# jdidion/atropos

Hardware: AMD Instinct MI355X
Metric: reads/s (whole node) 150 bp SE adapter-align (higher is better)
Workload: dtype int32

## Files before the change

### atropos_amd/csrc/piece_filter.hpp

```cpp
#ifndef ATR_PIECE_FILTER_HPP
#define ATR_PIECE_FILTER_HPP

#include "fast_work.hpp"
#include "pack_fast.hpp"

namespace atr {

#ifndef ATR_PIECE_PREFETCH_EARLY
#define ATR_PIECE_PREFETCH_EARLY 1
#endif
#ifndef ATR_PIECE_STASH
#define ATR_PIECE_STASH 1
#endif
#ifndef ATR_PIECE_WAVES
#if defined(ATR_SPEC) && defined(ATR_SPEC_ASCII)
#define ATR_PIECE_WAVES(NW) 2
#elif defined(ATR_SPEC)
#define ATR_PIECE_WAVES(NW) ((NW) <= 6 ? 4 : 3)
#else
#define ATR_PIECE_WAVES(NW) ((NW) <= 6 ? 4 : (NW) <= 8 ? 3 : 2)
#endif
#endif

constexpr int PIECE_QF = 2;
template <bool B> struct PieceBool { static constexpr bool value = B; };

__device__ __forceinline__ int lane_rank(uint64_t mask) {
    return (int)__builtin_amdgcn_mbcnt_hi((uint32_t)(mask >> 32), __builtin_amdgcn_mbcnt_lo((uint32_t)mask, 0u));
}

__device__ __forceinline__ void piece_emit(bool active, long long r, uint32_t ww, const uint32_t (&rec)[4], int m, uint4 *out,
                                           uint2 *list, uint4 *ldata, const uint32_t *nibs, int j0, uint32_t *s_lcur, uint32_t *s_hist,
                                           int nd = 8) {
    const bool open = active && window_valid(ww);
    if (active && !open) out[r] = make_uint4(rec[0], rec[1], rec[2], rec[3]);
    const uint64_t om = __ballot(open);
    if (om != 0ull) {
        uint32_t base = 0u;
        if ((threadIdx.x & 63) == 0) base = atomicAdd(s_lcur, (uint32_t)__popcll(om));
        base = __builtin_amdgcn_readfirstlane(base);
        const int lane = threadIdx.x & 63;
        const int off = window_lo(ww) - j0;
        const bool dense = nibs != nullptr && off >= 0 && off < 64 && band_stream_dwords(m) <= 8;
        if (open) {
            const uint32_t slot = base + (uint32_t)lane_rank(om);
            list[slot] = make_uint2((uint32_t)r, dense ? ww : (ww | PIECE_NODENSE));
            atomicAdd(&s_hist[window_bin(ww, m, true)], 1u);
            if (dense) {
                const int z = off >> 3;
                const uint32_t sh = 4u * (uint32_t)(off & 7);
                uint32_t raw[9], d[8];
#pragma unroll
                for (int k = 0; k < 9; ++k) raw[k] = z + k < nd ? nibs[(z + k) * 64 + lane] : 0u;
#pragma unroll
                for (int k = 0; k < 8; ++k) d[k] = sh ? ((raw[k] >> sh) | (raw[k + 1] << (32u - sh))) : raw[k];
                ldata[2 * (size_t)slot] = make_uint4(d[0], d[1], d[2], d[3]);
                ldata[2 * (size_t)slot + 1] = make_uint4(d[4], d[5], d[6], d[7]);
            }
        }
    }
}

template <int NW, bool RAGGED, int WW = 2>
__device__ __forceinline__ void piece_filter_body(const LocateParams &p, const FilterParams &fp_arg, const PieceParams &pp_arg,
                                                  const uint4 *__restrict__ planes, const int32_t *__restrict__ lens,
                                                  long long nreads, int max_len, uint4 *__restrict__ out, FastWork wk,
                                                  const uint8_t *__restrict__ ascii = nullptr, const uint8_t *tab = nullptr) {
#ifdef ATR_SPEC
    if (!RAGGED) max_len = spec::N;
#endif
#ifdef ATR_SPEC_ASCII
    static_assert(NW <= 8, "the fused ASCII entry keeps pass B's window in the LDS stash");
    constexpr int STRIDE = ATR_SPEC_STRIDE;
    constexpr int NPC = (15 + 64 * STRIDE + 1023) / 1024;
    constexpr int STAGE_BYTES = (64 * STRIDE + PACK_STAGE_SLACK + 15) & ~15;
    __shared__ __attribute__((aligned(16))) uint8_t s_stage[4][STAGE_BYTES];
    __shared__ uint8_t s_tab[256];
    s_tab[threadIdx.x] = tab[threadIdx.x];
    uint4 *planes_out = const_cast<uint4 *>(planes);
    const uint8_t *buf_end = ascii + nreads * STRIDE;
#endif
    const int n = RAGGED ? 32 * NW : max_len;
    __shared__ uint2 s_peq[16];
    __shared__ uint32_t s_spread[4][256];
    __shared__ uint32_t s_hist[FILTER_BINS];
    __shared__ uint32_t s_lcur, s_wcnt;
    constexpr int PW = 32 * WW, ND = 4 * WW;
#ifdef ATR_SPEC
    constexpr bool WIDE_OK = true;
#else
    constexpr bool WIDE_OK = WW == 3;
#endif
    static_assert(WW == 2 || WW == 3, "windows of 64 or 96 columns");
    __shared__ uint32_t s_nibs[4][ND][64];
    __shared__ uint32_t s_queue[4][PIECE_QF][64];
    constexpr bool STASH = ATR_PIECE_STASH != 0 && NW <= 8;
    __shared__ uint4 s_stash[STASH ? 4 : 1][STASH ? NW : 1][64];
    const Uniform u = make_uniform(p, round_up_rows_dev(p.m));
#ifndef ATR_SPEC
    __shared__ PieceParams s_pp;
    __shared__ FilterParams s_fp;
    for (int i = threadIdx.x; i < (int)(sizeof(PieceParams) / 4); i += 256) ((uint32_t *)&s_pp)[i] = ((const uint32_t *)&pp_arg)[i];
    for (int i = threadIdx.x; i < (int)(sizeof(FilterParams) / 4); i += 256) ((uint32_t *)&s_fp)[i] = ((const uint32_t *)&fp_arg)[i];
    const PieceParams &pp = s_pp;
    const FilterParams &fp = s_fp;
#else
    const PieceParams &pp = pp_arg;
    const FilterParams &fp = fp_arg;
#endif
    if (threadIdx.x < 16) s_peq[threadIdx.x] = make_uint2((uint32_t)fp_arg.peq[threadIdx.x], (uint32_t)(fp_arg.peq[threadIdx.x] >> 32));
    if (threadIdx.x < FILTER_BINS) s_hist[threadIdx.x] = 0;
    if (threadIdx.x == 0) { s_lcur = 0; s_wcnt = 0; }
    piece_spread_fill(s_spread);
    __syncthreads();

    const int lane = threadIdx.x & 63, wave = __builtin_amdgcn_readfirstlane((int)(threadIdx.x >> 6));
    const int mf = fp_arg.rows, T = u.m - mf;
    const uint32_t kreg = (uint32_t)u.k;
    const long long ntiles = (nreads + 63) >> 6;
    long long t0, t1;
    block_tiles(ntiles, t0, t1, wk.nused);
    uint2 *list = wk.tmp + t0 * 64;
    uint4 *ldata = wk.tdata + t0 * 128;
    uint32_t *wlist = wk.wide + t0 * 64;
    uint32_t (*queue)[64] = s_queue[wave];
    uint32_t *nibs = &s_nibs[wave][0][0];
    uint4 (*stash)[64] = s_stash[STASH ? wave : 0];

    auto pass_b = [&](int count) __attribute__((always_inline)) {
        const bool act = lane < count;
        const long long r = (long long)queue[0][lane];
        const uint32_t meta = queue[1][lane];
        const int j_e = act ? (int)(meta & 1023u) : 0, need = act ? (int)((meta >> 10) & 127u) : 0;
        const int nr = RAGGED ? (act ? (int)(meta >> 17) : 0) : max_len;
        uint32_t wp[4][WW];
        {
            const int b0 = j_e - PW + (STASH && RAGGED ? 32 * NW - nr : 0), w0 = b0 >> 5;
            uint4 g[WW + 1];
#pragma unroll
            for (int i = 0; i <= WW; ++i) g[i] = make_uint4(0u, 0u, 0u, 0u);
            if constexpr (STASH) {
                if (act) {
#pragma unroll
                    for (int i = 0; i <= WW; ++i) if (w0 + i >= 0 && w0 + i < NW) g[i] = stash[w0 + i][lane];
                }
            } else {
#ifndef ATR_X_NOGATHER
                const uint4 *tcur = planes + ((size_t)(r >> 6) * NW) * 64 + (r & 63);
                if (act) {
#pragma unroll
                    for (int i = 0; i <= WW; ++i) if (w0 + i >= 0 && w0 + i < NW) g[i] = tcur[(size_t)(w0 + i) * 64];
                }
#endif
            }
            const uint32_t sh = (uint32_t)(b0 & 31);
#pragma unroll
            for (int i = 0; i < WW; ++i) {
                wp[0][i] = __builtin_amdgcn_alignbit(g[i + 1].x, g[i].x, sh);
                wp[1][i] = __builtin_amdgcn_alignbit(g[i + 1].y, g[i].y, sh);
                wp[2][i] = __builtin_amdgcn_alignbit(g[i + 1].z, g[i].z, sh);
                wp[3][i] = __builtin_amdgcn_alignbit(g[i + 1].w, g[i].w, sh);
            }
        }
        const int W = min(PW, (wave_max_i32(need) + 7) & ~7);
        const int dw0 = ND - (W >> 3);
        uint32_t nb[ND];
#pragma unroll
        for (int d = 0; d < ND; ++d) {
            nb[d] = 0u;
            if (d >= dw0 - 1) nb[d] = piece_nibbles(s_spread, wp[0][d >> 2], wp[1][d >> 2], wp[2][d >> 2], wp[3][d >> 2], d & 3);
            nibs[d * 64 + lane] = nb[d];
        }
        const auto sweep_decide = [&](auto wc) __attribute__((always_inline)) {
        constexpr bool WD = decltype(wc)::value;
        FilterState F;
        filter_init(F, u, mf, WD);
        int vstart = 0;
        if (u.sr) {
            const bool zero0 = j_e - W <= 0;
            Uniform uf = u;
            uf.sr = false;
            FilterState G;
            filter_init(G, uf, mf, WD);
            if (!zero0) { F.pvl = G.pvl; F.pvh = G.pvh; F.score = G.score; }
            vstart = zero0 ? PW - j_e : 0;
        }
        uint2 ea[8], eb[8];
#pragma unroll
        for (int d = 0; d < ND; ++d) {
            if (d < dw0) continue;
            uint2 (&e)[8] = (d & 1) ? eb : ea;
            if (d == dw0) fetch_peq8(s_peq, nb[d], e);
            if (d + 1 < ND) fetch_peq8(s_peq, nb[d + 1], (d & 1) ? ea : eb);
            if (u.sr) {
#pragma unroll
                for (int b = 0; b < 8; ++b) if (8 * d + b < vstart) { e[b].x = ~0u; e[b].y = ~0u; }
            }
#pragma unroll
            for (int b = 0; b < 8; ++b) filter_step<WD>(F, e[b].x, e[b].y, kreg);
            if ((d & 3) == 3 && d + 1 < ND) filter_fold(F, j_e - PW + 8 * (d + 1), mf, kreg);
        }
        filter_fold(F, j_e, mf, kreg);
        uint32_t rec[4];
        const auto tm = [&](int jp) {
            const int rp = max(0, jp - (j_e - PW));
            return filter_tail_cmp(fp, T, rp, [&](int z) { return z < ND ? nibs[z * 64 + lane] : 0u; });
        };
        const auto dg = [&](int d) -> uint64_t {
            if constexpr (WW != 2 || WD) return ~0ull;
            const int o = d - (j_e - PW);
            if (o < 0 || o + u.m > PW) return ~0ull;
            uint64_t eq = 0ull;
#pragma unroll
            for (int c = 0; c < 4; ++c) {
                uint32_t lo = wp[c][0], hi = wp[c][1];
#pragma unroll
                for (int q = 0; q < 4; ++q) if (q != c && !fp.and_mode) { lo &= ~wp[q][0]; hi &= ~wp[q][1]; }
                eq |= ((((uint64_t)hi << 32) | lo) >> o) & fp.rowsel[c];
            }
            return ~eq & (u.m >= 64 ? ~0ull : (1ull << u.m) - 1ull);
        };
        const uint32_t ww = filter_decide_tm<WD>(F, u, fp, tm, nr, rec, 0, j_e == nr, dg, j_e - need, j_e < nr ? j_e - u.m : -0x10000);
        piece_emit(act, r, ww, rec, u.m, out, list, ldata, nibs, j_e - PW, &s_lcur, s_hist, ND);
        };
        if (mf > 32) {
            if constexpr (WIDE_OK) sweep_decide(PieceBool<true>{});
        } else {
            sweep_decide(PieceBool<false>{});
        }
    };

    int qn = 0;

#ifdef ATR_SPEC_ASCII
    uint4 ax[NPC];
    const auto ascii_edge = [&](long long tile) {
        const uint8_t *src = ascii + tile * 64 * STRIDE;
        const uint8_t *al = src - ((uintptr_t)src & 15);
        const long long need = (long long)((uintptr_t)src & 15) + (nreads - tile * 64 < 64 ? nreads - tile * 64 : 64) * STRIDE;
        return al < ascii || al + ((need + 15) & ~15ll) > buf_end;
    };
    const auto ascii_request = [&](long long tile) {
        if (ascii_edge(tile)) return;
        const uint8_t *src = ascii + tile * 64 * STRIDE;
        const uint8_t *al = src - ((uintptr_t)src & 15);
        const long long need = (long long)((uintptr_t)src & 15) + (nreads - tile * 64 < 64 ? nreads - tile * 64 : 64) * STRIDE;
#pragma unroll
        for (int u = 0; u < NPC; ++u) {
            const long long o = (long long)u * 1024 + (long long)lane * 16;
            ax[u] = o < need ? *(const uint4 *)(al + o) : make_uint4(0u, 0u, 0u, 0u);
        }
    };
    if (t0 + wave < t1) ascii_request(t0 + wave);
#else
    uint4 nx[NW];
    if (t0 + wave < t1) {
        const uint4 *tp = planes + (size_t)(t0 + wave) * NW * 64;
#pragma unroll
        for (int w = 0; w < NW; ++w) nx[w] = tp[w * 64 + lane];
    }
#endif
    for (long long tile = t0 + wave; tile < t1; tile += 4) {
        const long long r = tile * 64 + lane;
        const bool live = r < nreads;
        uint32_t pl[NW][4];
#ifdef ATR_SPEC_ASCII
        {
            uint8_t *stage = s_stage[wave];
            uint32_t mis;
            if (ascii_edge(tile)) {
                mis = pack_stage_tile(stage, ascii, STRIDE, nreads, tile, lane);
            } else {
                const uint8_t *src = ascii + tile * 64 * STRIDE;
                mis = (uint32_t)((uintptr_t)src & 15);
                const long long need = (long long)mis + (nreads - tile * 64 < 64 ? nreads - tile * 64 : 64) * STRIDE;
#pragma unroll
                for (int u = 0; u < NPC; ++u) {
                    const long long o = (long long)u * 1024 + (long long)lane * 16;
                    if (o < need) *(uint4 *)(stage + o) = ax[u];
                }
                __builtin_amdgcn_wave_barrier();
                __builtin_amdgcn_s_waitcnt(0);
            }
            if (tile + 4 < t1) ascii_request(tile + 4);
            __builtin_amdgcn_sched_barrier(0);
            const int np = live ? (RAGGED ? min(max(lens[r], 0), max_len) : max_len) : 0;
            const uint32_t rowoff = mis + (uint32_t)lane * (uint32_t)STRIDE;
            uint4 pk[NW];
            bool zero_seen = false;
            pack_planes_row_regs<NW>((const uint32_t *)stage, rowoff >> 2, rowoff & 3u, np, s_tab, pk, zero_seen);
            uint4 *tp = planes_out + (size_t)tile * NW * 64;
#pragma unroll
            for (int w = 0; w < NW; ++w) {
                tp[w * 64 + lane] = pk[w];
                pl[w][0] = pk[w].x; pl[w][1] = pk[w].y; pl[w][2] = pk[w].z; pl[w][3] = pk[w].w;
            }
        }
#else
#pragma unroll
        for (int w = 0; w < NW; ++w) { pl[w][0] = nx[w].x; pl[w][1] = nx[w].y; pl[w][2] = nx[w].z; pl[w][3] = nx[w].w; }
#if ATR_PIECE_PREFETCH_EARLY
        if (tile + 4 < t1) {
            const uint4 *tp = planes + (size_t)(tile + 4) * NW * 64;
#pragma unroll
            for (int w = 0; w < NW; ++w) nx[w] = tp[w * 64 + lane];
        }
        __builtin_amdgcn_sched_barrier(0);
#endif
#endif
        int nr = max_len, back = 0;
        constexpr int HWN = NW < PIECE_HEAD_WORDS ? NW : PIECE_HEAD_WORDS;
        uint32_t hpl[HWN][4];
#pragma unroll
        for (int w = 0; w < HWN; ++w)
#pragma unroll
            for (int c = 0; c < 4; ++c) hpl[w][c] = pl[w][c];
        if (RAGGED) {
            nr = live ? min(max(lens[r], 0), max_len) : 0;
            back = 32 * NW - nr;
            const int q = (back - 1) >> 5;
            const uint32_t sh = (uint32_t)(-back) & 31u;
            uint32_t x0[NW][4], x1[NW][4];
#pragma unroll
            for (int w = 0; w < NW; ++w)
#pragma unroll
                for (int c = 0; c < 4; ++c) x0[w][c] = x1[w][c] = 0u;
#pragma unroll
            for (int v = -1; v <= NW - 1; ++v) {
                const uint32_t sel = q == v ? ~0u : 0u;
#pragma unroll
                for (int w = 0; w < NW; ++w)
#pragma unroll
                    for (int c = 0; c < 4; ++c) {
                        if (w - v - 1 >= 0 && w - v - 1 < NW) x0[w][c] |= pl[w - v - 1 >= 0 && w - v - 1 < NW ? w - v - 1 : 0][c] & sel;
                        if (w - v >= 0 && w - v < NW) x1[w][c] |= pl[w - v >= 0 && w - v < NW ? w - v : 0][c] & sel;
                    }
            }
#pragma unroll
            for (int w = 0; w < NW; ++w)
#pragma unroll
                for (int c = 0; c < 4; ++c) pl[w][c] = __builtin_amdgcn_alignbit(x1[w][c], x0[w][c], sh);
        }
        uint32_t twp[4];
        {
            const int sh = n & 31;
#pragma unroll
            for (int q = 0; q < 4; ++q)
                twp[q] = sh == 0 ? pl[NW - 1][q] : __builtin_amdgcn_alignbit(pl[NW - 1][q], NW >= 2 ? pl[NW >= 2 ? NW - 2 : 0][q] : 0u, (uint32_t)sh);
        }
#ifdef ATR_SPEC
        const PieceScan S = piece_scan_spec<NW>(pl, twp, mf, T, u.k, hpl);
#else
        const PieceScan S = piece_scan<NW, (WW == 3 ? PIECE_NB : 5)>(pp, pl, twp, n, mf, T, u.k, hpl);
#endif
        const PieceTask pt = piece_task(S, back, nr, u.sr, u.m, u.k, piece_uniform(pp.head_cols));
        const bool exact = live && S.j_exact != 0 && u.m >= u.min_overlap;
        if (exact) {
            const int j = S.j_exact - back;
            out[r] = make_uint4((uint32_t)u.m << 16, (uint32_t)(j - u.m) | ((uint32_t)j << 16), (uint32_t)u.m, 0u);
        }
        const bool ovl = ATR_PIECE_OVERLAP_A != 0 && live && S.ovl != 0 && !exact;
        if (ovl) out[r] = make_uint4((uint32_t)S.ovl << 16, (uint32_t)(nr - S.ovl) | ((uint32_t)nr << 16), (uint32_t)S.ovl, 0u);
        const bool flagged = live && pt.flagged && !exact;
        if (piece_uniform(pp.aonly) != 0) {
            if (live && !flagged && !exact && !ovl) out[r] = make_uint4(0xFFFF0000u, 0u, 0u, 0u);
            const int wlo = pt.full ? 0 : pt.j_e - pt.need, whi = pt.full ? nr : pt.j_e;
            const uint32_t ww = flagged ? window_word(wlo, whi, whi == nr, u.m, false) : 0u;
            const uint32_t none[4] = {0xFFFF0000u, 0u, 0u, 0u};
            piece_emit(flagged, r, ww, none, u.m, out, list, ldata, nullptr, 0, &s_lcur, s_hist);
            continue;
        }
        const int need = pt.need;
        const bool narrow = flagged && !pt.full && need <= piece_uniform(pp.narrow), wide = flagged && !narrow;
        if (live && !flagged && !exact && !ovl) out[r] = make_uint4(0xFFFF0000u, 0u, 0u, 0u);
        const uint32_t meta = (uint32_t)pt.j_e | ((uint32_t)need << 10) | (RAGGED ? (uint32_t)nr << 17 : 0u);
        {
            const uint64_t wm = __ballot(wide);
            if (wm != 0ull) {
                uint32_t base = 0u;
                if (lane == 0) base = atomicAdd(&s_wcnt, (uint32_t)__popcll(wm));
                base = __builtin_amdgcn_readfirstlane(base);
                if (wide) wlist[(long long)base + lane_rank(wm)] = (uint32_t)r;
            }
        }
#if !ATR_PIECE_PREFETCH_EARLY && !defined(ATR_SPEC_ASCII)
        __builtin_amdgcn_sched_barrier(0);
        if (tile + 4 < t1) {
            const uint4 *tp = planes + (size_t)(tile + 4) * NW * 64;
#pragma unroll
            for (int w = 0; w < NW; ++w) nx[w] = tp[w * 64 + lane];
        }
#endif
        {
            const uint64_t nm = __ballot(narrow);
            const int cnt = (int)__popcll(nm), rank = lane_rank(nm);
            const int room = 64 - qn;
            const auto put = [&](int slot) {
                queue[0][slot] = (uint32_t)r; queue[1][slot] = meta;
                if constexpr (STASH) {
#pragma unroll
                    for (int w = 0; w < NW; ++w) stash[w][slot] = make_uint4(pl[w][0], pl[w][1], pl[w][2], pl[w][3]);
                }
            };
            if (narrow && rank < room) put(qn + rank);
            if (cnt >= room) {
                __builtin_amdgcn_fence(__ATOMIC_RELEASE, "wavefront");
                pass_b(64);
                __builtin_amdgcn_fence(__ATOMIC_RELEASE, "wavefront");
                if (narrow && rank >= room) put(rank - room);
                qn = cnt - room;
            } else {
                qn += cnt;
            }
        }
    }
    __builtin_amdgcn_fence(__ATOMIC_RELEASE, "wavefront");
    if (qn > 0) pass_b(qn);
    __threadfence_block();
    __syncthreads();
    {
        const long long total = (long long)s_wcnt;
        for (long long base = (long long)wave * 64; base < total; base += 256) {
            const bool act = base + lane < total;
            const long long r = act ? (long long)wlist[base + lane] : t0 * 64;
            const uint4 *bp = planes + ((size_t)(r >> 6) * NW) * 64 + (r & 63);
            const uint4 *tp = bp;
            const size_t tstride = 64;
            const int nl = RAGGED ? (act ? min(max(lens[r], 0), max_len) : 0) : max_len;
            const int nhi = RAGGED ? wave_max_i32(nl) : max_len;
            const auto full_sweep = [&](auto wc) __attribute__((always_inline)) {
            constexpr bool WD = decltype(wc)::value;
            FilterState F;
            filter_init(F, u, mf, WD);
            int j = 0;
#pragma clang loop unroll(disable)
            for (int c = 0; c < NW; ++c) {
                if (j >= nhi) break;
                const uint4 v = tp[(size_t)c * tstride];
#pragma clang loop unroll(disable)
                for (int d = 0; d < 4; ++d) {
                    if (j >= nhi) break;
                    uint2 e[8];
                    fetch_peq8(s_peq, piece_nibbles(s_spread, v.x, v.y, v.z, v.w, d), e);
#pragma unroll
                    for (int b = 0; b < 8; ++b)
                        if (j + b < nl) filter_step<WD>(F, e[b].x, e[b].y, kreg);
                    j += 8;
                }
                filter_fold(F, min(j, nl), mf, kreg);
            }
            uint32_t rec[4];
            const auto tm = [&](int jp) {
                return filter_tail_cmp(fp, T, jp, [&](int z) { return read_dword_planes((const uint32_t *)bp, NW, z, s_spread); });
            };
            const uint32_t ww = filter_decide_tm<WD>(F, u, fp, tm, nl, rec, 0, true);
            piece_emit(act, r, ww, rec, u.m, out, list, ldata, nullptr, 0, &s_lcur, s_hist);
            };
            if (mf > 32) {
                if constexpr (WIDE_OK) full_sweep(PieceBool<true>{});
            } else {
                full_sweep(PieceBool<false>{});
            }
        }
    }
    __syncthreads();
    fused_hist_flush(wk, s_hist);
    if (threadIdx.x == 0) wk.lcount[blockIdx.x] = s_lcur;
}

}
#endif
```

### atropos_amd/csrc/piece_kernels.hip

```cpp
#include "locate_fast.hpp"
#include "piece_filter.hpp"
#include "jit.hpp"

namespace atr {

void launch_fast_scan(FastWork wk, hipStream_t st);
int launch_fast_dp(const atr_aligner *a, const uint4 *packed, const int32_t *lens, long long nreads, int nchunks,
                   int max_len, uint4 *out, FastWork wk, const LinkedArgs *la, int idx, int count, hipStream_t st, bool planes, bool one_stream);

template <int NW, bool RAGGED, int WW>
__global__ __launch_bounds__(256) __attribute__((amdgpu_waves_per_eu(ATR_PIECE_WAVES(NW), 8))) void piece_filter_kernel(
    const LocateParams p, const FilterParams fp, const PieceParams pp, const uint4 *__restrict__ planes,
    const int32_t *__restrict__ lens, long long nreads, int max_len, uint4 *__restrict__ out, FastWork wk) {
    piece_filter_body<NW, RAGGED, WW>(p, fp, pp, planes, lens, nreads, max_len, out, wk);
}

__global__ __launch_bounds__(256) void piece_scatter_kernel(long long nreads, int m, FastWork wk) {
    __shared__ uint32_t s_cur[FILTER_BINS + 1], s_tmp[256];
    const long long ntiles = (nreads + 63) >> 6;
    long long t0, t1;
    block_tiles(ntiles, t0, t1, wk.nused);
    const uint2 *list = wk.tmp + t0 * 64;
    const uint32_t count = wk.lcount[blockIdx.x];
    const uint32_t mine = threadIdx.x < FILTER_BINS ? wk.counts[(size_t)blockIdx.x * FILTER_BINS + threadIdx.x] : 0u;
    const uint2 first = threadIdx.x < count ? list[threadIdx.x] : make_uint2(0u, 0u);
    if (wk.fused) {
        fused_bin_bases(wk, s_cur, s_tmp);
        if (threadIdx.x < FILTER_BINS) s_cur[threadIdx.x] += mine;
    } else if (threadIdx.x < FILTER_BINS) s_cur[threadIdx.x] = fast_slot0(wk, threadIdx.x);
    __syncthreads();
    for (uint32_t i = threadIdx.x; i < count; i += 256) {
        const uint2 e = i == threadIdx.x ? first : list[i];
        const uint32_t slot = atomicAdd(&s_cur[window_bin(e.y & ~PIECE_NODENSE, m, true)], 1u);
        wk.order[slot] = e;
        wk.dref[slot] = (uint32_t)(t0 * 64) + i;
    }
}

template <int NW, bool RAGGED, int WW>
static int piece_resident_blocks() {
    static thread_local int cached_dev = -1, cached = 0;
    int dev = 0;
    if (hipGetDevice(&dev) != hipSuccess) return 1024;
    if (dev != cached_dev) {
        int per_cu = 0, cus = 0;
        if (hipOccupancyMaxActiveBlocksPerMultiprocessor(&per_cu, piece_filter_kernel<NW, RAGGED, WW>, 256, 0) != hipSuccess || per_cu < 1) per_cu = 2;
        if (hipDeviceGetAttribute(&cus, hipDeviceAttributeMultiprocessorCount, dev) != hipSuccess || cus < 1) cus = 256;
        cached = std::min(FAST_BLOCKS, per_cu * cus);
        cached_dev = dev;
    }
    return cached;
}

template <int NW, int WW>
static void launch_piece_filter_w(const atr_aligner *a, const FilterParams &fp, const PieceParams &pp, const uint4 *planes,
                                  const int32_t *lens, long long nreads, int max_len, uint4 *out, FastWork &wk, hipStream_t st) {
    const long long want = ((nreads + 63) / 64 + 3) / 4;
    if (lens) {
        wk.nused = (int)std::max<long long>(1, std::min<long long>(piece_resident_blocks<NW, true, WW>(), want));
        hipLaunchKernelGGL((piece_filter_kernel<NW, true, WW>), dim3(wk.nused), dim3(256), 0, st, a->p, fp, pp, planes, lens, nreads, max_len, out, wk);
    } else {
        wk.nused = (int)std::max<long long>(1, std::min<long long>(piece_resident_blocks<NW, false, WW>(), want));
        hipLaunchKernelGGL((piece_filter_kernel<NW, false, WW>), dim3(wk.nused), dim3(256), 0, st, a->p, fp, pp, planes, lens, nreads, max_len, out, wk);
    }
}
template <int NW>
static void launch_piece_filter(const atr_aligner *a, const FilterParams &fp, const PieceParams &pp, const uint4 *planes,
                                const int32_t *lens, long long nreads, int max_len, uint4 *out, FastWork &wk, hipStream_t st) {
    if (pp.window > PIECE_WINDOW || pp.nb > 5 || fp.rows > 32) launch_piece_filter_w<NW, 3>(a, fp, pp, planes, lens, nreads, max_len, out, wk, st);
    else launch_piece_filter_w<NW, 2>(a, fp, pp, planes, lens, nreads, max_len, out, wk, st);
}

int piece_ragged_len(int max_len) { return 32 * ((max_len + 31) / 32); }
bool piece_applies(const atr_aligner *a, int max_len, FilterParams *fp_out, PieceParams *pp_out) {
    if (!a->filterable || max_len < 1) return false;
    const FilterParams &fp = aligner_piece_filter_params(a);
    PieceParams pp;
    if (!piece_params(a->codes, a->p.m, fp.rows, a->p.k, a->flags, a->wildcard_ref || a->wildcard_query,
                      a->table_kind == ATR_TABLE_CUSTOM, fp.thr_row, max_len, pp, a->p.thr, a->p.min_overlap, fp.cert, a->p.indel)) return false;
    const int nw = (max_len + 31) / 32;
    if (nw < 3 || nw > 10) return false;
    if (fp_out) *fp_out = fp;
    if (pp_out) *pp_out = pp;
    return true;
}

static const jit::SpecKernel *piece_spec_for(const atr_aligner *a, const FilterParams &fp, const PieceParams &pp, bool ragged,
                                             int max_len, long long nreads, bool force, int ascii_stride = 0) {
    const int pol = jit::policy();
    if (pol == 0) return nullptr;
    const int nw = (max_len + 31) / 32;
    a->planes_seen += nreads;
    const bool compile = force || pol == 1 || a->planes_seen >= jit::min_reads();
    return jit::spec_kernel(a, fp, pp, nw, ragged, ragged ? 32 * nw : max_len, compile, ascii_stride);
}

static bool tail_spec_enabled() {
    const char *x = getenv("ATR_TAIL_SPEC");
    return !(x && x[0] == '0');
}

int prepare_locate_planes(const atr_aligner *a, int max_len, bool ragged) {
    FilterParams fp;
    PieceParams pp;
    if (!piece_applies(a, ragged ? piece_ragged_len(max_len) : max_len, &fp, &pp)) return 0;
    return piece_spec_for(a, fp, pp, ragged, max_len, 0, true) != nullptr ? 1 : 0;
}

int launch_planes_prepass(const atr_aligner *a, const uint4 *planes, const int32_t *lens, long long nreads, int max_len,
                          uint4 *out, void *work, hipStream_t st, int grid_div, PlanesCall *pc) {
    FilterParams fp;
    PieceParams pp;
    if (!piece_applies(a, lens ? piece_ragged_len(max_len) : max_len, &fp, &pp)) return (int)hipErrorInvalidValue;
    FastWork wk = fast_carve(work, nreads);
    wk.lpw = nreads <= 8192 ? 0 : 64;
    const int nw = (max_len + 31) / 32;
    const jit::SpecKernel *sk = piece_spec_for(a, fp, pp, lens != nullptr, max_len, nreads, false);
    wk.fused = fast_fused_scan() ? 1 : 0;
    if (wk.fused) {
        const hipError_t rc = hipMemsetAsync(wk.chunks, 0, (size_t)wk.nbins * 4, st);
        if (rc != hipSuccess) return (int)rc;
    }
    if (sk) {
        const long long want = ((nreads + 63) / 64 + 3) / 4;
        wk.nused = (int)std::max<long long>(1, std::min<long long>(std::max(1, sk->resident / std::max(1, grid_div)), want));
        const hipError_t rc = jit::spec_launch(sk, wk.nused, planes, lens, nreads, max_len, out, wk, st);
        if (rc != hipSuccess) return (int)rc;
    } else {
        switch (nw) {
        case 3: launch_piece_filter<3>(a, fp, pp, planes, lens, nreads, max_len, out, wk, st); break;
        case 4: launch_piece_filter<4>(a, fp, pp, planes, lens, nreads, max_len, out, wk, st); break;
        case 5: launch_piece_filter<5>(a, fp, pp, planes, lens, nreads, max_len, out, wk, st); break;
        case 6: launch_piece_filter<6>(a, fp, pp, planes, lens, nreads, max_len, out, wk, st); break;
        case 7: launch_piece_filter<7>(a, fp, pp, planes, lens, nreads, max_len, out, wk, st); break;
        case 8: launch_piece_filter<8>(a, fp, pp, planes, lens, nreads, max_len, out, wk, st); break;
        case 9: launch_piece_filter<9>(a, fp, pp, planes, lens, nreads, max_len, out, wk, st); break;
        default: launch_piece_filter<10>(a, fp, pp, planes, lens, nreads, max_len, out, wk, st); break;
        }
    }
    pc->wk = wk;
    pc->nw = nw;
    pc->tail = sk ? (void *)sk->tail : nullptr;
    return (int)hipGetLastError();
}

int launch_planes_tail(const atr_aligner *a, const uint4 *planes, const int32_t *lens, long long nreads, int max_len, uint4 *out,
                       const PlanesCall &pc, hipStream_t st, bool one_stream) {
    FastWork wk = pc.wk;
    if (!wk.fused) launch_fast_scan(wk, st);
    hipLaunchKernelGGL(piece_scatter_kernel, dim3(wk.nused), dim3(256), 0, st, nreads, a->p.m, wk);
    if (pc.tail && !one_stream && tail_spec_enabled()) {
        {
            const bool small = nreads <= 65536;
            const int win_blocks = (int)std::max<long long>(1, std::min<long long>((nreads + 3) / 4, 1024));
            const int band_blocks = (int)std::max<long long>(1, std::min<long long>(small ? (nreads + 3) / 4 : (nreads + 255) / 256, 4096));
            const hipError_t rc = jit::tail_launch((hipFunction_t)pc.tail, win_blocks, band_blocks, planes, lens, pc.nw, max_len, out, wk, st);
            return rc != hipSuccess ? (int)rc : (int)hipGetLastError();
        }
    }
    return launch_fast_dp(a, planes, lens, nreads, pc.nw, max_len, out, wk, nullptr, 0, 1, st, true, one_stream);
}

int launch_locate_planes_shared(const atr_aligner *a, const uint4 *planes, const int32_t *lens, long long nreads, int max_len,
                                uint4 *out, void *work, hipStream_t st, int grid_div, bool one_stream) {
    PlanesCall pc;
    const int rc = launch_planes_prepass(a, planes, lens, nreads, max_len, out, work, st, grid_div, &pc);
    if (rc != 0) return rc;
    return launch_planes_tail(a, planes, lens, nreads, max_len, out, pc, st, one_stream);
}

int launch_locate_ascii_fused(const atr_aligner *a, const uint8_t *ascii, long long row_stride, const int32_t *lens, long long nreads,
                              int max_len, const uint8_t table[256], uint4 *planes, uint4 *out, void *work, hipStream_t st) {
    FilterParams fp;
    PieceParams pp;
    if (!piece_applies(a, lens ? piece_ragged_len(max_len) : max_len, &fp, &pp)) return 1;
    const int nw = (max_len + 31) / 32;
    static const bool off = [] { const char *x = getenv("ATR_ASCII_FUSED"); return x && x[0] == '0'; }();
    if (off || nw > 8 || row_stride < max_len || row_stride > 256 || ((uintptr_t)ascii & 1)) return 1;
    const jit::SpecKernel *sk = piece_spec_for(a, fp, pp, lens != nullptr, max_len, nreads, jit::policy() != 0, (int)row_stride);
    if (!sk) return 1;
    FastWork wk = fast_carve(work, nreads);
    wk.lpw = nreads <= 8192 ? 0 : 64;
    wk.fused = fast_fused_scan() ? 1 : 0;
    if (wk.fused) {
        const hipError_t rc = hipMemsetAsync(wk.chunks, 0, (size_t)wk.nbins * 4, st);
        if (rc != hipSuccess) return (int)rc;
    }
    const long long want = ((nreads + 63) / 64 + 3) / 4;
    wk.nused = (int)std::max<long long>(1, std::min<long long>(sk->resident, want));
    const hipError_t rc = jit::spec_launch_ascii(sk, wk.nused, ascii, lens, nreads, max_len, out, wk, planes, table, st);
    if (rc != hipSuccess) return (int)rc;
    PlanesCall pc;
    pc.wk = wk;
    pc.nw = nw;
    pc.tail = (void *)sk->tail;
    return launch_planes_tail(a, planes, lens, nreads, max_len, out, pc, st, false);
}

int launch_locate_planes(const atr_aligner *a, const uint4 *planes, const int32_t *lens, long long nreads, int max_len, uint4 *out,
                         void *work, hipStream_t st) {
    return launch_locate_planes_shared(a, planes, lens, nreads, max_len, out, work, st, 1, false);
}

}
```

### atropos_amd/csrc/piece_spec.hip

```cpp
#include "piece_filter.hpp"

#define ATR_SPEC_WAVES (atr::spec::PP.nb > 5 ? (ATR_PIECE_WAVES(ATR_SPEC_NW) < 3 ? ATR_PIECE_WAVES(ATR_SPEC_NW) : 3) : ATR_PIECE_WAVES(ATR_SPEC_NW))

#ifdef ATR_SPEC_ASCII
extern "C" __global__ __launch_bounds__(256) __attribute__((amdgpu_waves_per_eu(ATR_SPEC_WAVES, 8)))
void atr_piece_spec(const uint8_t *__restrict__ ascii, const int32_t *__restrict__ lens, long long nreads, int max_len,
                    uint4 *__restrict__ out, atr::FastWork wk, uint4 *__restrict__ planes, const atr::PackTableArg tab) {
    atr::piece_filter_body<ATR_SPEC_NW, ATR_SPEC_RAGGED != 0, (atr::spec::PP.window > atr::PIECE_WINDOW ? 3 : 2)>(atr::spec::P, atr::spec::FP, atr::spec::PP, planes, lens, nreads,
                                                             max_len, out, wk, ascii, tab.t);
}
#else
extern "C" __global__ __launch_bounds__(256) __attribute__((amdgpu_waves_per_eu(ATR_SPEC_WAVES, 8)))
void atr_piece_spec(const uint4 *__restrict__ planes, const int32_t *__restrict__ lens, long long nreads, int max_len,
                    uint4 *__restrict__ out, atr::FastWork wk) {
    atr::piece_filter_body<ATR_SPEC_NW, ATR_SPEC_RAGGED != 0, (atr::spec::PP.window > atr::PIECE_WINDOW ? 3 : 2)>(atr::spec::P, atr::spec::FP, atr::spec::PP, planes, lens, nreads,
                                                             max_len, out, wk);
}
#endif

#ifdef ATR_TAIL_SPEC
#include "tail_spec.hip"
#endif
```

Baseline: 24.48 billion.

## Split narrow queue by read kind, queue wide reads per wave, balance drain across waves

Narrow candidates are split into two queues. Reads whose window ends at the read end get a fixed-offset stash holding only WW+1 planes, which skips the variable-offset gather. Wide reads are queued per wave in LDS and swept in batches of 64 instead of going through a global list after a block barrier. Leftover work in all queues is pooled across the four waves with prefix sums, so the final drain is balanced. The extra LDS can lower blocks per CU, so the waves-per-EU hint is capped by an LDS-derived limit, and an env var can cap the grid.

```diff
diff --git a/atropos_amd/csrc/piece_filter.hpp b/atropos_amd/csrc/piece_filter.hpp
--- a/atropos_amd/csrc/piece_filter.hpp
+++ b/atropos_amd/csrc/piece_filter.hpp
@@ -22,8 +22,34 @@
 #endif
 #endif
 
+#ifndef ATR_PIECE_KINDS
+#define ATR_PIECE_KINDS 1
+#endif
+#ifndef ATR_PIECE_WIDE_QUEUE
+#define ATR_PIECE_WIDE_QUEUE 1
+#endif
+#ifndef ATR_PIECE_DRAIN
+#define ATR_PIECE_DRAIN 1
+#endif
+#if defined(ATR_SPEC) && !defined(ATR_SPEC_ASCII)
+#define ATR_PIECE_QUEUES_OK 1
+#else
+#define ATR_PIECE_QUEUES_OK 0
+#endif
+
 constexpr int PIECE_QF = 2;
 template <bool B> struct PieceBool { static constexpr bool value = B; };
+template <int K> struct PieceKind { static constexpr int value = K; };
+
+constexpr int piece_kinds_lds(int nw, int ww) {
+    return 128 + 4096 + 1024 + 4096 * ww  + 4096  + 4096 * nw + 4096 * (ww + 1)  + 1024  + 256;
+}
+constexpr bool piece_kinds_on(int nw, int ww) {
+    return ATR_PIECE_QUEUES_OK != 0 && ATR_PIECE_KINDS != 0 && ATR_PIECE_STASH != 0 && nw <= 8 && piece_kinds_lds(nw, ww) <= 65536;
+}
+constexpr int piece_lds_blocks(int nw, int ww) {
+    return piece_kinds_on(nw, ww) ? 163840 / piece_kinds_lds(nw, ww) : 8;
+}
 
 __device__ __forceinline__ int lane_rank(uint64_t mask) {
     return (int)__builtin_amdgcn_mbcnt_hi((uint32_t)(mask >> 32), __builtin_amdgcn_mbcnt_lo((uint32_t)mask, 0u));
@@ -93,9 +119,22 @@
 #endif
     static_assert(WW == 2 || WW == 3, "windows of 64 or 96 columns");
     __shared__ uint32_t s_nibs[4][ND][64];
-    __shared__ uint32_t s_queue[4][PIECE_QF][64];
     constexpr bool STASH = ATR_PIECE_STASH != 0 && NW <= 8;
+    constexpr bool KINDS = piece_kinds_on(NW, WW);
+    constexpr bool WIDEQ = ATR_PIECE_QUEUES_OK != 0 && ATR_PIECE_WIDE_QUEUE != 0;
+    constexpr bool DRAIN = ATR_PIECE_QUEUES_OK != 0 && ATR_PIECE_DRAIN != 0;
+    constexpr int NK = KINDS ? 2 : 1;
+    __shared__ uint32_t s_queue[4][NK][PIECE_QF][64];
     __shared__ uint4 s_stash[STASH ? 4 : 1][STASH ? NW : 1][64];
+#ifdef ATR_SPEC
+    constexpr int K1B0 = spec::N - PW;
+#else
+    constexpr int K1B0 = 32 * NW - PW;
+#endif
+    constexpr int K1W0 = (K1B0 - (K1B0 < 0 ? 31 : 0)) / 32;
+    __shared__ uint4 s_stash1[KINDS ? 4 : 1][KINDS ? WW + 1 : 1][KINDS ? 64 : 1];
+    __shared__ uint32_t s_wq[WIDEQ ? 4 : 1][WIDEQ ? 64 : 1];
+    __shared__ int s_left[DRAIN ? 4 : 1][3];
     const Uniform u = make_uniform(p, round_up_rows_dev(p.m));
 #ifndef ATR_SPEC
     __shared__ PieceParams s_pp;
@@ -123,26 +162,29 @@
     uint2 *list = wk.tmp + t0 * 64;
     uint4 *ldata = wk.tdata + t0 * 128;
     uint32_t *wlist = wk.wide + t0 * 64;
-    uint32_t (*queue)[64] = s_queue[wave];
     uint32_t *nibs = &s_nibs[wave][0][0];
-    uint4 (*stash)[64] = s_stash[STASH ? wave : 0];
-
-    auto pass_b = [&](int count) __attribute__((always_inline)) {
-        const bool act = lane < count;
-        const long long r = (long long)queue[0][lane];
-        const uint32_t meta = queue[1][lane];
+
+    auto pass_b = [&](auto kc, bool act, int ow, int sl) __attribute__((always_inline)) {
+        constexpr int KIND = decltype(kc)::value, QI = KIND == 1 ? 1 : 0;
+        const long long r = (long long)s_queue[ow][QI][0][sl];
+        const uint32_t meta = s_queue[ow][QI][1][sl];
         const int j_e = act ? (int)(meta & 1023u) : 0, need = act ? (int)((meta >> 10) & 127u) : 0;
         const int nr = RAGGED ? (act ? (int)(meta >> 17) : 0) : max_len;
         uint32_t wp[4][WW];
         {
-            const int b0 = j_e - PW + (STASH && RAGGED ? 32 * NW - nr : 0), w0 = b0 >> 5;
+            const int b0 = KIND == 1 ? K1B0 : j_e - PW + (STASH && RAGGED ? 32 * NW - nr : 0), w0 = b0 >> 5;
             uint4 g[WW + 1];
 #pragma unroll
             for (int i = 0; i <= WW; ++i) g[i] = make_uint4(0u, 0u, 0u, 0u);
-            if constexpr (STASH) {
+            if constexpr (KIND == 1) {
                 if (act) {
 #pragma unroll
-                    for (int i = 0; i <= WW; ++i) if (w0 + i >= 0 && w0 + i < NW) g[i] = stash[w0 + i][lane];
+                    for (int i = 0; i <= WW; ++i) if (K1W0 + i >= 0 && K1W0 + i < NW) g[i] = s_stash1[KINDS ? ow : 0][KINDS ? i : 0][sl];
+                }
+            } else if constexpr (STASH) {
+                if (act) {
+#pragma unroll
+                    for (int i = 0; i <= WW; ++i) if (w0 + i >= 0 && w0 + i < NW) g[i] = s_stash[ow][w0 + i][sl];
                 }
             } else {
 #ifndef ATR_X_NOGATHER
@@ -220,7 +262,8 @@
             }
             return ~eq & (u.m >= 64 ? ~0ull : (1ull << u.m) - 1ull);
         };
-        const uint32_t ww = filter_decide_tm<WD>(F, u, fp, tm, nr, rec, 0, j_e == nr, dg, j_e - need, j_e < nr ? j_e - u.m : -0x10000);
+        const bool have_last = KIND < 0 ? j_e == nr : KIND == 1;
+        const uint32_t ww = filter_decide_tm<WD>(F, u, fp, tm, nr, rec, 0, have_last, dg, j_e - need, !have_last ? j_e - u.m : -0x10000);
         piece_emit(act, r, ww, rec, u.m, out, list, ldata, nibs, j_e - PW, &s_lcur, s_hist, ND);
         };
         if (mf > 32) {
@@ -230,7 +273,49 @@
         }
     };
 
-    int qn = 0;
+    auto wide_sweep = [&](bool act, long long r) __attribute__((always_inline)) {
+        const uint4 *bp = planes + ((size_t)(r >> 6) * NW) * 64 + (r & 63);
+        const uint4 *tp = bp;
+        const size_t tstride = 64;
+        const int nl = RAGGED ? (act ? min(max(lens[r], 0), max_len) : 0) : max_len;
+        const int nhi = RAGGED ? wave_max_i32(nl) : max_len;
+        const auto full_sweep = [&](auto wc) __attribute__((always_inline)) {
+        constexpr bool WD = decltype(wc)::value;
+        FilterState F;
+        filter_init(F, u, mf, WD);
+        int j = 0;
+#pragma clang loop unroll(disable)
+        for (int c = 0; c < NW; ++c) {
+            if (j >= nhi) break;
+            const uint4 v = tp[(size_t)c * tstride];
+#pragma clang loop unroll(disable)
+            for (int d = 0; d < 4; ++d) {
+                if (j >= nhi) break;
+                uint2 e[8];
+                fetch_peq8(s_peq, piece_nibbles(s_spread, v.x, v.y, v.z, v.w, d), e);
+#pragma unroll
+                for (int b = 0; b < 8; ++b)
+                    if (j + b < nl) filter_step<WD>(F, e[b].x, e[b].y, kreg);
+                j += 8;
+            }
+            filter_fold(F, min(j, nl), mf, kreg);
+        }
+        uint32_t rec[4];
+        const auto tm = [&](int jp) {
+            return filter_tail_cmp(fp, T, jp, [&](int z) { return read_dword_planes((const uint32_t *)bp, NW, z, s_spread); });
+        };
+        const uint32_t ww = filter_decide_tm<WD>(F, u, fp, tm, nl, rec, 0, true);
+        piece_emit(act, r, ww, rec, u.m, out, list, ldata, nullptr, 0, &s_lcur, s_hist);
+        };
+        if (mf > 32) {
+            if constexpr (WIDE_OK) full_sweep(PieceBool<true>{});
+        } else {
+            full_sweep(PieceBool<false>{});
+        }
+    };
+
+    int qn[NK] = {};
+    int wqn = 0;
 
 #ifdef ATR_SPEC_ASCII
     uint4 ax[NPC];
@@ -374,7 +459,7 @@
         const bool narrow = flagged && !pt.full && need <= piece_uniform(pp.narrow), wide = flagged && !narrow;
         if (live && !flagged && !exact && !ovl) out[r] = make_uint4(0xFFFF0000u, 0u, 0u, 0u);
         const uint32_t meta = (uint32_t)pt.j_e | ((uint32_t)need << 10) | (RAGGED ? (uint32_t)nr << 17 : 0u);
-        {
+        if constexpr (!WIDEQ) {
             const uint64_t wm = __ballot(wide);
             if (wm != 0ull) {
                 uint32_t base = 0u;
@@ -391,75 +476,115 @@
             for (int w = 0; w < NW; ++w) nx[w] = tp[w * 64 + lane];
         }
 #endif
-        {
-            const uint64_t nm = __ballot(narrow);
+        const auto enqueue = [&](auto kc, bool mine, int &qk) __attribute__((always_inline)) {
+            constexpr int KIND = decltype(kc)::value, QI = KIND == 1 ? 1 : 0;
+            const uint64_t nm = __ballot(mine);
             const int cnt = (int)__popcll(nm), rank = lane_rank(nm);
-            const int room = 64 - qn;
+            const int room = 64 - qk;
             const auto put = [&](int slot) {
-                queue[0][slot] = (uint32_t)r; queue[1][slot] = meta;
-                if constexpr (STASH) {
-#pragma unroll
-                    for (int w = 0; w < NW; ++w) stash[w][slot] = make_uint4(pl[w][0], pl[w][1], pl[w][2], pl[w][3]);
+                s_queue[wave][QI][0][slot] = (uint32_t)r; s_queue[wave][QI][1][slot] = meta;
+                if constexpr (KIND == 1) {
+#pragma unroll
+                    for (int i = 0; i <= WW; ++i) {
+                        const int w = K1W0 + i;
+                        const int wc = w >= 0 && w < NW ? w : 0;
+                        if (w >= 0 && w < NW) s_stash1[KINDS ? wave : 0][KINDS ? i : 0][slot] = make_uint4(pl[wc][0], pl[wc][1], pl[wc][2], pl[wc][3]);
+                    }
+                } else if constexpr (STASH) {
+#pragma unroll
+                    for (int w = 0; w < NW; ++w) s_stash[wave][w][slot] = make_uint4(pl[w][0], pl[w][1], pl[w][2], pl[w][3]);
                 }
             };
-            if (narrow && rank < room) put(qn + rank);
+            if (mine && rank < room) put(qk + rank);
             if (cnt >= room) {
                 __builtin_amdgcn_fence(__ATOMIC_RELEASE, "wavefront");
-                pass_b(64);
+                pass_b(kc, true, wave, lane);
                 __builtin_amdgcn_fence(__ATOMIC_RELEASE, "wavefront");
-                if (narrow && rank >= room) put(rank - room);
-                qn = cnt - room;
+                if (mine && rank >= room) put(rank - room);
+                qk = cnt - room;
             } else {
-                qn += cnt;
+                qk += cnt;
+            }
+        };
+        if constexpr (KINDS) {
+            const bool k1 = pt.j_e == nr;
+            enqueue(PieceKind<0>{}, narrow && !k1, qn[0]);
+            enqueue(PieceKind<1>{}, narrow && k1, qn[NK - 1]);
+        } else {
+            enqueue(PieceKind<-1>{}, narrow, qn[0]);
+        }
+        if constexpr (WIDEQ) {
+            const uint64_t wm = __ballot(wide);
+            if (wm != 0ull) {
+                const int cnt = (int)__popcll(wm), rank = lane_rank(wm);
+                const int room = 64 - wqn;
+                if (wide && rank < room) s_wq[wave][wqn + rank] = (uint32_t)r;
+                if (cnt >= room) {
+                    __builtin_amdgcn_fence(__ATOMIC_RELEASE, "wavefront");
+                    wide_sweep(true, (long long)s_wq[wave][lane]);
+                    __builtin_amdgcn_fence(__ATOMIC_RELEASE, "wavefront");
+                    if (wide && rank >= room) s_wq[wave][rank - room] = (uint32_t)r;
+                    wqn = cnt - room;
+                } else {
+                    wqn += cnt;
+                }
             }
         }
     }
     __builtin_amdgcn_fence(__ATOMIC_RELEASE, "wavefront");
-    if (qn > 0) pass_b(qn);
-    __threadfence_block();
-    __syncthreads();
-    {
-        const long long total = (long long)s_wcnt;
-        for (long long base = (long long)wave * 64; base < total; base += 256) {
-            const bool act = base + lane < total;
-            const long long r = act ? (long long)wlist[base + lane] : t0 * 64;
-            const uint4 *bp = planes + ((size_t)(r >> 6) * NW) * 64 + (r & 63);
-            const uint4 *tp = bp;
-            const size_t tstride = 64;
-            const int nl = RAGGED ? (act ? min(max(lens[r], 0), max_len) : 0) : max_len;
-            const int nhi = RAGGED ? wave_max_i32(nl) : max_len;
-            const auto full_sweep = [&](auto wc) __attribute__((always_inline)) {
-            constexpr bool WD = decltype(wc)::value;
-            FilterState F;
-            filter_init(F, u, mf, WD);
-            int j = 0;
-#pragma clang loop unroll(disable)
-            for (int c = 0; c < NW; ++c) {
-                if (j >= nhi) break;
-                const uint4 v = tp[(size_t)c * tstride];
-#pragma clang loop unroll(disable)
-                for (int d = 0; d < 4; ++d) {
-                    if (j >= nhi) break;
-                    uint2 e[8];
-                    fetch_peq8(s_peq, piece_nibbles(s_spread, v.x, v.y, v.z, v.w, d), e);
-#pragma unroll
-                    for (int b = 0; b < 8; ++b)
-                        if (j + b < nl) filter_step<WD>(F, e[b].x, e[b].y, kreg);
-                    j += 8;
-                }
-                filter_fold(F, min(j, nl), mf, kreg);
-            }
-            uint32_t rec[4];
-            const auto tm = [&](int jp) {
-                return filter_tail_cmp(fp, T, jp, [&](int z) { return read_dword_planes((const uint32_t *)bp, NW, z, s_spread); });
-            };
-            const uint32_t ww = filter_decide_tm<WD>(F, u, fp, tm, nl, rec, 0, true);
-            piece_emit(act, r, ww, rec, u.m, out, list, ldata, nullptr, 0, &s_lcur, s_hist);
-            };
-            if (mf > 32) {
-                if constexpr (WIDE_OK) full_sweep(PieceBool<true>{});
+    if constexpr (DRAIN) {
+        if (lane == 0) {
+            s_left[wave][0] = qn[0];
+            s_left[wave][1] = KINDS ? qn[NK - 1] : 0;
+            s_left[wave][2] = WIDEQ ? wqn : 0;
+        }
+        __threadfence_block();
+        __syncthreads();
+        int pre[3][5];
+#pragma unroll
+        for (int c = 0; c < 3; ++c) {
+            pre[c][0] = 0;
+#pragma unroll
+            for (int v = 0; v < 4; ++v) pre[c][v + 1] = pre[c][v] + s_left[v][c];
+        }
+        const int wtotal = WIDEQ ? pre[2][4] : (int)s_wcnt;
+        const int rw = (wtotal + 63) >> 6, r0 = (pre[0][4] + 63) >> 6, r1 = (pre[1][4] + 63) >> 6;
+        for (int g = wave; g < rw + r0 + r1; g += 4) {
+            const int c = g < rw ? 2 : g < rw + r0 ? 0 : 1;
+            const int idx = 64 * (g - (c == 2 ? 0 : c == 0 ? rw : rw + r0)) + lane;
+            const int p1 = c == 2 ? pre[2][1] : c == 0 ? pre[0][1] : pre[1][1], p2 = c == 2 ? pre[2][2] : c == 0 ? pre[0][2] : pre[1][2];
+            const int p3 = c == 2 ? pre[2][3] : c == 0 ? pre[0][3] : pre[1][3], p4 = c == 2 ? wtotal : c == 0 ? pre[0][4] : pre[1][4];
+            const bool act = idx < p4;
+            const int ow = act ? (idx >= p1) + (idx >= p2) + (idx >= p3) : wave;
+            const int sl = act ? idx - (ow == 0 ? 0 : ow == 1 ? p1 : ow == 2 ? p2 : p3) : lane;
+            if (c == 2) {
+                long long r = t0 * 64;
+                if constexpr (WIDEQ) { if (act) r = (long long)s_wq[ow][sl]; }
+                else { if (act) r = (long long)wlist[idx]; }
+                wide_sweep(act, r);
+            } else if (c == 0) {
+                if constexpr (KINDS) pass_b(PieceKind<0>{}, act, ow, sl);
+                else pass_b(PieceKind<-1>{}, act, ow, sl);
             } else {
-                full_sweep(PieceBool<false>{});
+                if constexpr (KINDS) pass_b(PieceKind<1>{}, act, ow, sl);
+            }
+        }
+    } else {
+        if constexpr (KINDS) {
+            if (qn[0] > 0) pass_b(PieceKind<0>{}, lane < qn[0], wave, lane);
+            if (qn[NK - 1] > 0) pass_b(PieceKind<1>{}, lane < qn[NK - 1], wave, lane);
+        } else {
+            if (qn[0] > 0) pass_b(PieceKind<-1>{}, lane < qn[0], wave, lane);
+        }
+        if constexpr (WIDEQ) {
+            if (wqn > 0) wide_sweep(lane < wqn, lane < wqn ? (long long)s_wq[wave][lane] : t0 * 64);
+        } else {
+            __threadfence_block();
+            __syncthreads();
+            const long long total = (long long)s_wcnt;
+            for (long long base = (long long)wave * 64; base < total; base += 256) {
+                const bool act = base + lane < total;
+                wide_sweep(act, act ? (long long)wlist[base + lane] : t0 * 64);
             }
         }
     }
diff --git a/atropos_amd/csrc/piece_kernels.hip b/atropos_amd/csrc/piece_kernels.hip
--- a/atropos_amd/csrc/piece_kernels.hip
+++ b/atropos_amd/csrc/piece_kernels.hip
@@ -100,6 +100,12 @@
     return !(x && x[0] == '0');
 }
 
+static int piece_grid_cap() {
+    const char *x = getenv("ATR_PIECE_GRID");
+    const int v = x ? atoi(x) : 0;
+    return v >= 1 ? v : 0x7fffffff;
+}
+
 int prepare_locate_planes(const atr_aligner *a, int max_len, bool ragged) {
     FilterParams fp;
     PieceParams pp;
@@ -124,6 +130,7 @@
     if (sk) {
         const long long want = ((nreads + 63) / 64 + 3) / 4;
         wk.nused = (int)std::max<long long>(1, std::min<long long>(std::max(1, sk->resident / std::max(1, grid_div)), want));
+        wk.nused = std::min(wk.nused, piece_grid_cap());
         const hipError_t rc = jit::spec_launch(sk, wk.nused, planes, lens, nreads, max_len, out, wk, st);
         if (rc != hipSuccess) return (int)rc;
     } else {
diff --git a/atropos_amd/csrc/piece_spec.hip b/atropos_amd/csrc/piece_spec.hip
--- a/atropos_amd/csrc/piece_spec.hip
+++ b/atropos_amd/csrc/piece_spec.hip
@@ -1,6 +1,8 @@
 #include "piece_filter.hpp"
 
-#define ATR_SPEC_WAVES (atr::spec::PP.nb > 5 ? (ATR_PIECE_WAVES(ATR_SPEC_NW) < 3 ? ATR_PIECE_WAVES(ATR_SPEC_NW) : 3) : ATR_PIECE_WAVES(ATR_SPEC_NW))
+#define ATR_SPEC_WAVES_REGS (atr::spec::PP.nb > 5 ? (ATR_PIECE_WAVES(ATR_SPEC_NW) < 3 ? ATR_PIECE_WAVES(ATR_SPEC_NW) : 3) : ATR_PIECE_WAVES(ATR_SPEC_NW))
+#define ATR_SPEC_WW (atr::spec::PP.window > atr::PIECE_WINDOW ? 3 : 2)
+#define ATR_SPEC_WAVES (ATR_SPEC_WAVES_REGS < atr::piece_lds_blocks(ATR_SPEC_NW, ATR_SPEC_WW) ? ATR_SPEC_WAVES_REGS : atr::piece_lds_blocks(ATR_SPEC_NW, ATR_SPEC_WW))
 
 #ifdef ATR_SPEC_ASCII
 extern "C" __global__ __launch_bounds__(256) __attribute__((amdgpu_waves_per_eu(ATR_SPEC_WAVES, 8)))
```

Result: slower. 23.92 billion (-2.3%).
